# rmazzier/OpenSetGaitRecognition_PCAA

Hardware: AMD Instinct MI355X
Metric: gait sequences/sec (train step) (higher is better)
Workload: dtype bf16; 1 GPU; PCAA V4 train step (enc+dec+disc fwd/bwd, WGAN-GP, Chamfer, 2x Adam), B=64/GPU T=30 N=128 C=4 K=8, BASELINE config[1]; global_batch=64, precision=bf16, parallelism=dp1, sync_bn=False, finite_loss=True, hip_graph=False, decoder_update=fused wgrad+adam

## Files before the change

### include/pcaa_hip.h

```cpp
#ifndef PCAA_HIP_H
#define PCAA_HIP_H

#include <stddef.h>

#ifdef __cplusplus
extern "C" {
#endif

#define PCAA_ABI_VERSION 20

#define PCAA_OK 0
#define PCAA_ERR_INVALID_ARG 1
#define PCAA_ERR_LAUNCH 2

#define PCAA_F32 0
#define PCAA_BF16 1
#define PCAA_SPLIT_F16 2

#define PCAA_LAYOUT_KC 0
#define PCAA_LAYOUT_RC 1

#define PCAA_ACT_NONE 0
#define PCAA_ACT_ELU 1

const char* pcaa_last_error(void);
int pcaa_abi_version(void);

int pcaa_gemm(int math,
              const void* A, int a_dtype, int a_layout, long lda,
              const void* B, int b_dtype, int b_layout, long ldb,
              void* C, int c_dtype, long ldc,
              int M, int N, int K,
              const float* bias, double* colstats, int nrep,
              int split_k, int accumulate, void* stream);

int pcaa_gemm_num_splits(int math, int K, int split_k);
int pcaa_gemm_group_rc_f32(int n, const void* const* A, const void* const* B, void* const* C, const int* M,
                           const int* N, const int* K, const int* split_k, void* stream);
int pcaa_gemm_group_rc_f32_slabs(int n, const void* const* A, const void* const* B, void* const* slabs, const int* M,
                                 const int* N, const int* K, const int* split_k, void* stream);
int pcaa_gemm_v2_enable(int on);
int pcaa_gemm_slabs(int math,
// ... 85 lines not shown
                         float* scale, float* shift, float* mean, float* rstd, int ch, unsigned* counter);
int pcaa_bn_tail_arm_bwd(const double* stats, int nrep, long count, const float* gamma,
                         const float* mean, const float* rstd,
                         float* coef, float* dgamma, float* dbeta, int ch, unsigned* counter);
int pcaa_bn_tail_pending(void);
int pcaa_bn_tail_disarm(void);
int pcaa_bn_bwd_dy_fused(const void* da, const float* dpool, int group_rows, float pool_scale,
                         const void* y, void* dy, int dtype, const float* scale, const float* shift,
                         const float* coef, long rows, int ch, void* stream);

int pcaa_bias_act(float* y, const float* bias, int act, long rows, int cols, void* stream);
int pcaa_elu_bwd_from_out(const float* da, const float* a, float* dz, long n, void* stream);
int pcaa_colsum(const float* x, float* out, long rows, int cols, void* stream);
int pcaa_sum(const float* x, long n, float scale, float* out, void* stream);
int pcaa_rowsum(const float* x, float* out, long rows, int cols, float scale, void* stream);
int pcaa_scale_by_device_scalar(const float* x, const float* s, float* out, long n, void* stream);
int pcaa_scale_rows(const float* x, const float* s, float* out, long rows, int cols, void* stream);
int pcaa_prior_sample(const float* z0, const float* means, const long long* gt, int B, int K, int D,
                      float* z, float* onehot, void* stream);
int pcaa_pack_points(const float* src, long sb, long sc, long st, long sn,
                     float* dst, int B, int C, int T, int N, void* stream);

int pcaa_gather_rows(const void* src, long n_src_rows, long row_bytes, const long long* idx, void* dst,
                     long n_rows, int* err_flag, void* stream);

int pcaa_dtc_im2col(const float* a, float* col, int B, int T, int Cin, int dilation, void* stream);
int pcaa_dtc_col2im(const float* dcol, float* da, int B, int T, int Cin, int dilation, void* stream);

int pcaa_chamfer_fwd_bwd(const float* preds, long p_sb, long p_sc, long p_st, long p_sn,
                         const float* gts, long g_sb, long g_sc, long g_st, long g_sn,
                         int B, int T, int N, int C, float* frame_loss,
                         float* dpreds, long d_sb, long d_sc, long d_st, long d_sn,
                         float grad_scale, const float* grad_per_b, void* stream);
int pcaa_cross_entropy(const float* logits, const long long* target, int B, int K,
                       float* loss, float* dlogits, float grad_scale, long long* preds,
                       int* err_flag, void* stream);

int pcaa_disc_forward(const float* x, const float* label, int B, int K,
                      const float* W1, const float* b1, const float* W2, const float* b2,
                      const float* W3, const float* b3, float* out, void* stream);
int pcaa_disc_backward(const float* x, const float* label, int B, int K,
                       const float* W1, const float* b1, const float* W2, const float* b2,
                       const float* W3, const float* b3, const float* gout,
                       float* dx, float* dlabel,
                       float* dW1, float* db1, float* dW2, float* db2, float* dW3, float* db3,
                       float* workspace, size_t workspace_bytes, void* stream);
int pcaa_disc_backward_backward(const float* x, const float* label, int B, int K,
                                const float* W1, const float* b1, const float* W2, const float* b2,
                                const float* W3, const float* b3, const float* gout, const float* gbar,
                                float* dx2, float* dlabel2, float* dgout,
                                float* dW1, float* db1, float* dW2, float* db2, float* dW3, float* db3,
                                float* workspace, size_t workspace_bytes, void* stream);
size_t pcaa_disc_workspace_bytes(int B, int K);
int pcaa_disc_wgan_gp(const float* z, const float* fv, const float* label, const float* alphas,
                      int B, int K,
                      const float* W1, const float* b1, const float* W2, const float* b2,
                      const float* W3, const float* b3, float gp_weight, float* losses,
                      float* dW1, float* db1, float* dW2, float* db2, float* dW3, float* db3,
                      float* dz, float* workspace, size_t workspace_bytes, void* stream);

int pcaa_joint_likelihood(const float* x, const float* means, int B, int K, int D, double* lik,
                          void* stream);
int pcaa_kvote(const double* lik, const long long* preds, double threshold, int k, int n_labels,
               int n_classes, int n_windows, long long* out, void* stream);

int pcaa_skinny_supported(int M, int N, int K);
// ... 104 lines not shown
                   float* dW1, float* db1, float* dWh, float* dbh, float* dW2, float* db2, float* dWg,
                   float* dbg, float* dx4, int B, int K, void* stream);

int pcaa_gemm_split3_supported(int M, int N, int K);
int pcaa_gemm_split3(const void* A, const void* B, int layout, long lda, long ldb, float* C, long ldc, int M,
                     int N, int K, double* colstats, int nrep, float out_scale, void* stream);
int pcaa_gemm_split3_num_splits(int K, int split_k);
int pcaa_gemm_slabs_split3(const void* A, const void* B, int layout, long lda, long ldb, float* slabs,
                           long slab_stride, int M, int N, int K, int split_k, float out_scale, void* stream);
int pcaa_split_f16(const float* src, void* dst_img, long rows, int ch, int transpose, float img_scale, void* stream);
int pcaa_set_range_flag(int* dev_flag);
int pcaa_bn_act_fwd_split(const float* y, void* a_img, const float* scale, const float* shift, long rows,
                          int ch, float img_scale, void* stream);
int pcaa_bn_bwd_dy_fused_split(const float* da, const float* dpool, int group_rows, float pool_scale,
                               const float* y, void* dy_img, const float* scale, const float* shift,
                               const float* coef, long rows, int ch, float img_scale, void* stream);

int pcaa_orced_heads_supported(int B, int K, int d_in, int d_lat);
int pcaa_orced_heads_fwd(const float* x4, const float* Wmu, const float* bmu, const float* Wlv, const float* blv,
                         const float* eps, const float* Wc, const float* bc, float* mu, float* logvar, float* sup_fv,
                         float* logits, int B, int K, int d_in, int d_lat, void* stream);
int pcaa_orced_heads_bwd(const float* x4, const float* eps, const float* logvar, const float* sup_fv,
                         const float* Wmu, const float* Wlv, const float* Wc, const float* d_logits,
                         const float* d_sup, const float* d_mu, const float* d_logvar, float* ws, float* dWmu,
                         float* dbmu, float* dWlv, float* dblv, float* dWc, float* dbc, float* dx4, int B, int K,
                         int d_in, int d_lat, void* stream);
int pcaa_orced_kl(const float* mu, const float* logvar, const float* mu_k, float* loss, float* d_mu,
                  float* d_logvar, float* d_muk, float gscale, int B, int d_lat, void* stream);

int pcaa_adam_step(float* param, const float* grad, float* exp_avg, float* exp_avg_sq, long n,
                   float lr, float beta1, float beta2, float eps, int step, float grad_scale,
                   int max_blocks, void* stream);
int pcaa_adam_advance(int* step_dev, float* coef_dev, float lr, float beta1, float beta2, void* stream);
int pcaa_adam_step_dev(float* param, const float* grad, float* exp_avg, float* exp_avg_sq, long n,
                       float beta1, float beta2, float eps, const float* coef_dev, float grad_scale,
                       int max_blocks, void* stream);
int pcaa_adam_step_dev_g16(float* param, const void* grad_bf16, float* exp_avg, float* exp_avg_sq, long n,
                           float beta1, float beta2, float eps, const float* coef_dev, float grad_scale,
                           int max_blocks, void* stream);

#ifdef __cplusplus
}
#endif
#endif
```

### opensetgaitrecognition_pcaa_amd/csrc/elementwise.hip

```cpp
#include <stdarg.h>

#include "common.h"
#include "bn_tail.h"

static thread_local char g_err[512] = "";
void pcaa_set_error(const char* fmt, ...) {
  va_list ap;
  va_start(ap, fmt);
  vsnprintf(g_err, sizeof(g_err), fmt, ap);
  va_end(ap);
}
extern "C" const char* pcaa_last_error(void) { return g_err; }
static thread_local int* g_range_flag = nullptr;
int* pcaa_range_flag_ptr() { return g_range_flag; }
extern "C" int pcaa_set_range_flag(int* dev_flag) { g_range_flag = dev_flag; return PCAA_OK; }
extern "C" int pcaa_abi_version(void) { return PCAA_ABI_VERSION; }

namespace {

constexpr int ROWS_PER_BLOCK = 128;

inline bool ch_ok(int ch) {
  if (ch < 4 || ch > 1024 || (ch & 3)) return false;
  const int q = ch >> 2;
// ... 505 lines not shown
  const long stride = (long)gridDim.x * 256;
  for (long q0 = (long)blockIdx.x * 256 + threadIdx.x; q0 < nq; q0 += stride * U) {
    f32x4 pv[U], gv[U], mv[U], vv[U];
#pragma unroll
    for (int u = 0; u < U; ++u) {
      const long q = q0 + u * stride;
      if (q < nq) { pv[u] = load4(p + q * 4); gv[u] = load4(g + q * 4); mv[u] = load4(m + q * 4); vv[u] = load4(v + q * 4); }
    }
#pragma unroll
    for (int u = 0; u < U; ++u) {
      const long q = q0 + u * stride;
      if (q >= nq) break;
#pragma unroll
      for (int e = 0; e < 4; ++e) {
        float pe = pv[u][e], me = mv[u][e], ve = vv[u][e];
        adam_update(pe, me, ve, gv[u][e] * grad_scale, b1, b2, eps, step_size, inv_bc2_sqrt);
        pv[u][e] = pe; mv[u][e] = me; vv[u][e] = ve;
      }
      store4(p + q * 4, pv[u]);
      store4(m + q * 4, mv[u]);
      store4(v + q * 4, vv[u]);
    }
  }
  if (blockIdx.x == 0 && threadIdx.x < (n & 3)) {
    const long i = (nq << 2) + threadIdx.x;
    float pp = p[i], mm = m[i], vv = v[i];
    adam_update(pp, mm, vv, (float)g[i] * grad_scale, b1, b2, eps, step_size, inv_bc2_sqrt);
    m[i] = mm;
    v[i] = vv;
    p[i] = pp;
  }
}

__global__ void adam_coef_kernel(int* __restrict__ step, float* __restrict__ coef, float lr, float b1, float b2) {
  const int t = *step + 1;
  *step = t;
  const double bc1 = 1.0 - pow((double)b1, (double)t);
  const double bc2 = 1.0 - pow((double)b2, (double)t);
  coef[0] = (float)((double)lr / bc1);
  coef[1] = (float)(1.0 / sqrt(bc2));
}

inline int grid_for(long work_items, int per_block = 256, int cap = 256 * 8) {
  long g = cdiv(work_items, per_block);
  if (g < 1) g = 1;
  if (g > cap) g = cap;
  return (int)g;
}

inline int col_invariant_grid(long nquads, int qpr) {
  int a = qpr, b = 256;
  while (b) { const int t = a % b; a = b; b = t; }
  const int unit = qpr / a;
  long g = cdiv(nquads, 256);
  if (g > 2048) g = 2048;
  g = cdiv(g, unit) * unit;
  return (int)g;
}

}

extern "C" int pcaa_bn_finalize(const double* stats, int nrep, long count, const float* lin_bias,
                                const float* gamma, const float* beta, float* running_mean,
                                float* running_var, long long* num_batches_tracked, float momentum,
                                float eps, float* scale, float* shift, float* mean, float* rstd,
                                int ch, void* stream) {
  PCAA_CHECK_ARG(stats && gamma && beta && scale && shift && mean && rstd, "pcaa_bn_finalize: null pointer");
  PCAA_CHECK_ARG(nrep >= 1 && count >= 1 && ch >= 1, "pcaa_bn_finalize: bad sizes");
  PCAA_CHECK_ARG((running_mean == nullptr) == (running_var == nullptr), "pcaa_bn_finalize: running stats must come together");
  const double unbias = count > 1 ? (double)count / (double)(count - 1) : 1.0;
  hipLaunchKernelGGL(bn_finalize_kernel, dim3((unsigned)cdiv(ch, 256)), dim3(256), 0, as_stream(stream),
                     stats, nrep, 1.0 / (double)count, unbias, lin_bias, gamma, beta, running_mean,
                     running_var, num_batches_tracked, momentum, eps, scale, shift, mean, rstd, ch);
// ... 499 lines not shown
                                      int max_blocks, void* stream) {
  PCAA_CHECK_ARG(param && grad_bf16 && exp_avg && exp_avg_sq && coef_dev && n >= 1 && max_blocks >= 0,
                 "pcaa_adam_step_dev_g16: bad args");
  PCAA_CHECK_ARG(((uintptr_t)param % 16) == 0 && ((uintptr_t)grad_bf16 % 8) == 0 && ((uintptr_t)exp_avg % 16) == 0 &&
                 ((uintptr_t)exp_avg_sq % 16) == 0, "pcaa_adam_step_dev_g16: buffers must be 16-B (gradient: 8-B) aligned");
  const bf16_t* g = reinterpret_cast<const bf16_t*>(grad_bf16);
  const int cap = max_blocks > 0 ? max_blocks : 256 * 16;
  if (cap <= 1024)
    hipLaunchKernelGGL((adam_kernel<4, bf16_t>), dim3(grid_for(n >> 4, 256, cap)), dim3(256), 0, as_stream(stream), param, g,
                       exp_avg, exp_avg_sq, n, beta1, beta2, eps, 0.f, 0.f, grad_scale, coef_dev);
  else
    hipLaunchKernelGGL((adam_kernel<1, bf16_t>), dim3(grid_for(n >> 2, 256, cap)), dim3(256), 0, as_stream(stream), param, g,
                       exp_avg, exp_avg_sq, n, beta1, beta2, eps, 0.f, 0.f, grad_scale, coef_dev);
  PCAA_RETURN_LAUNCH_STATUS("pcaa_adam_step_dev_g16");
}

extern "C" int pcaa_adam_step(float* param, const float* grad, float* exp_avg, float* exp_avg_sq, long n,
                              float lr, float beta1, float beta2, float eps, int step, float grad_scale,
                              int max_blocks, void* stream) {
  PCAA_CHECK_ARG(param && grad && exp_avg && exp_avg_sq && n >= 1 && step >= 1 && max_blocks >= 0,
                 "pcaa_adam_step: bad args");
  const double bc1 = 1.0 - pow((double)beta1, (double)step);
  const double bc2 = 1.0 - pow((double)beta2, (double)step);
  return launch_adam(param, grad, exp_avg, exp_avg_sq, n, beta1, beta2, eps, (float)((double)lr / bc1),
                     (float)(1.0 / sqrt(bc2)), nullptr, grad_scale, max_blocks, stream, "pcaa_adam_step");
}

extern "C" int pcaa_adam_advance(int* step_dev, float* coef_dev, float lr, float beta1, float beta2, void* stream) {
  PCAA_CHECK_ARG(step_dev && coef_dev, "pcaa_adam_advance: bad args");
  hipLaunchKernelGGL(adam_coef_kernel, dim3(1), dim3(1), 0, as_stream(stream), step_dev, coef_dev, lr, beta1, beta2);
  PCAA_RETURN_LAUNCH_STATUS("pcaa_adam_advance");
}

extern "C" int pcaa_adam_step_dev(float* param, const float* grad, float* exp_avg, float* exp_avg_sq, long n,
                                  float beta1, float beta2, float eps, const float* coef_dev, float grad_scale,
                                  int max_blocks, void* stream) {
  PCAA_CHECK_ARG(param && grad && exp_avg && exp_avg_sq && coef_dev && n >= 1 && max_blocks >= 0,
                 "pcaa_adam_step_dev: bad args");
  return launch_adam(param, grad, exp_avg, exp_avg_sq, n, beta1, beta2, eps, 0.f, 0.f, coef_dev, grad_scale,
                     max_blocks, stream, "pcaa_adam_step_dev");
}
```

### opensetgaitrecognition_pcaa_amd/csrc/losses.hip

```cpp
#include "common.h"

namespace {

constexpr int MAXC = 8;
constexpr int CH_THREADS = 256;

__global__ __launch_bounds__(CH_THREADS) void chamfer_kernel(
    const float* __restrict__ preds, long p_sb, long p_sc, long p_st, long p_sn,
    const float* __restrict__ gts, long g_sb, long g_sc, long g_st, long g_sn,
    int T, int N, int C, float* __restrict__ frame_loss,
    float* __restrict__ dpreds, long d_sb, long d_sc, long d_st, long d_sn,
    float grad_scale, const float* __restrict__ grad_per_b) {
  extern __shared__ __attribute__((aligned(16))) float sm[];
  float* sg = sm;
  float* sp = sg + (long)N * MAXC;
  float* rg = sp + (long)N * MAXC;
  float* rp = rg + N;
  int* nn = reinterpret_cast<int*>(rp + N);
  __shared__ float red[CH_THREADS / 64];

  const int frame = blockIdx.x;
  const int b = frame / T, t = frame - b * T;
  const float* pb = preds + b * p_sb + t * p_st;
  const float* gb = gts + b * g_sb + t * g_st;
// ... 31 lines not shown
    float best = 3.4e38f;
    int bi = 0;
    for (int o = 0; o < N; ++o) {
      float dot = 0.f;
#pragma unroll
      for (int c = 0; c < MAXC; ++c) dot = fmaf(other[o * MAXC + c], v[c], dot);
      const float P = (dir1 ? (rother[o] + rme) : (rme + rother[o])) - 2.f * dot;
      if (P < best) { best = P; bi = o; }
    }
    loss += best;
    nn[item] = bi;
  }
  loss = wave_sum(loss);
  if ((threadIdx.x & 63) == 0) red[threadIdx.x >> 6] = loss;
  __syncthreads();
  if (threadIdx.x == 0) {
    float tot = 0.f;
    for (int i = 0; i < CH_THREADS / 64; ++i) tot += red[i];
    frame_loss[frame] = tot;
  }
  if (dpreds) {
    __syncthreads();
    float* db = dpreds + b * d_sb + t * d_st;
    for (int e = threadIdx.x; e < N * C; e += CH_THREADS) {
      const int c = e / N, n = e - c * N;
      const float pv = sp[n * MAXC + c];
      float g = 2.f * w * (pv - sg[nn[n] * MAXC + c]);
      for (int i = 0; i < N; ++i)
        if (nn[N + i] == n) g += 2.f * w * (pv - sg[i * MAXC + c]);
      db[c * d_sc + n * d_sn] = g;
    }
  }
}

__global__ __launch_bounds__(256) void cross_entropy_kernel(const float* __restrict__ logits,
                                                            const long long* __restrict__ target, int B,
                                                            int K, float* loss, float* dlogits,
                                                            float grad_scale, long long* preds, int* err_flag) {
  __shared__ double red[4];
  double acc = 0.0;
  for (int r = threadIdx.x; r < B; r += 256) {
    const float* x = logits + (long)r * K;
    float mx = x[0];
    for (int k = 1; k < K; ++k) mx = fmaxf(mx, x[k]);
    float se = 0.f;
    for (int k = 0; k < K; ++k) se += expf(x[k] - mx);
    const float inv = 1.f / se;
    int am = 0;
    float pbest = -1.f;
    long long tg = target ? target[r] : 0;
    if (tg < 0 || tg >= K) {
      if (err_flag) *err_flag = 1;
      tg = 0;
    }
    for (int k = 0; k < K; ++k) {
      const float pk = expf(x[k] - mx) / se;
      if (pk > pbest) { pbest = pk; am = k; }
      if (dlogits) dlogits[(long)r * K + k] = grad_scale * (expf(x[k] - mx) * inv - (k == tg ? 1.f : 0.f)) / (float)B;
    }
    if (preds) preds[r] = am;
    if (target) acc += (double)(logf(se) + mx - x[tg]);
  }
  acc = wave_sum_d(acc);
  if ((threadIdx.x & 63) == 0) red[threadIdx.x >> 6] = acc;
  __syncthreads();
  if (threadIdx.x == 0 && loss) loss[0] = (float)((red[0] + red[1] + red[2] + red[3]) / B);
}

}

extern "C" int pcaa_chamfer_fwd_bwd(const float* preds, long p_sb, long p_sc, long p_st, long p_sn,
                                    const float* gts, long g_sb, long g_sc, long g_st, long g_sn,
                                    int B, int T, int N, int C, float* frame_loss, float* dpreds,
                                    long d_sb, long d_sc, long d_st, long d_sn, float grad_scale,
                                    const float* grad_per_b, void* stream) {
  PCAA_CHECK_ARG(preds && gts && frame_loss, "pcaa_chamfer_fwd_bwd: null pointer");
  PCAA_CHECK_ARG(B >= 1 && T >= 1 && N >= 1 && C >= 1 && C <= MAXC, "pcaa_chamfer_fwd_bwd: need 1<=C<=%d (C=%d)", MAXC, C);
  const size_t lds = ((size_t)2 * N * MAXC + 4 * (size_t)N) * sizeof(float);
  PCAA_CHECK_ARG(lds <= 150 * 1024, "pcaa_chamfer_fwd_bwd: N=%d too large for one LDS tile", N);
  if (lds > 64 * 1024) {
    hipError_t e = hipFuncSetAttribute(reinterpret_cast<const void*>(chamfer_kernel),
                                       hipFuncAttributeMaxDynamicSharedMemorySize, (int)lds);
    if (e != hipSuccess) { pcaa_set_error("pcaa_chamfer_fwd_bwd: cannot raise LDS limit: %s", hipGetErrorString(e)); return PCAA_ERR_LAUNCH; }
  }
  hipLaunchKernelGGL(chamfer_kernel, dim3((unsigned)(B * T)), dim3(CH_THREADS), lds, as_stream(stream),
                     preds, p_sb, p_sc, p_st, p_sn, gts, g_sb, g_sc, g_st, g_sn, T, N, C, frame_loss,
                     dpreds, d_sb, d_sc, d_st, d_sn, grad_scale, grad_per_b);
  PCAA_RETURN_LAUNCH_STATUS("pcaa_chamfer_fwd_bwd");
}

extern "C" int pcaa_cross_entropy(const float* logits, const long long* target, int B, int K, float* loss,
                                  float* dlogits, float grad_scale, long long* preds, int* err_flag,
                                  void* stream) {
  PCAA_CHECK_ARG(logits && B >= 1 && K >= 1, "pcaa_cross_entropy: bad args");
  PCAA_CHECK_ARG(target || (!loss && !dlogits), "pcaa_cross_entropy: loss/grad need targets");
  hipLaunchKernelGGL(cross_entropy_kernel, dim3(1), dim3(256), 0, as_stream(stream), logits, target, B, K,
                     loss, dlogits, grad_scale, preds, err_flag);
  PCAA_RETURN_LAUNCH_STATUS("pcaa_cross_entropy");
}
```

### opensetgaitrecognition_pcaa_amd/ops.py

```python
import ctypes
import os

import torch

from . import _lib
from ._lib import ACT_ELU, ACT_NONE, KC, PCAA_BF16, PCAA_F32, RC, check

PCAA_SPLIT_F16 = 2

NREP = 16
BN_EPS = 1e-5
BN_MOMENTUM = 0.1


def _p(t):
    return None if t is None else t.data_ptr()


_raw_stream = getattr(torch._C, "_cuda_getCurrentRawStream", None)
_raw_device = getattr(torch._C, "_cuda_getDevice", None)


def _s():
    if _raw_stream is not None and _raw_device is not None:
# ... 1428 lines not shown
    D = sup_fv.shape[1]
    k, n_votes, n_runs = int(k), int(n_votes), run_start.numel() - 1
    if (sup_fv.shape[0] != nw or means.shape[1] != D or win_stream.numel() != nw or win_j.numel() != nw
            or vote_pos.numel() != nw or k < 1 or tuple(hist_lik.shape) != tuple(hist_pred.shape)
            or hist_lik.shape[1] != k or not 0 <= n_votes <= nw or not (1 <= n_runs <= nw or nw == 0)):
        raise ValueError("stream_score: shapes do not describe one tick")
    dev = logits.device
    preds = torch.empty(nw, dtype=torch.int64, device=dev)
    lik = torch.empty(nw, dtype=torch.float64, device=dev)
    votes = torch.empty(n_votes, dtype=torch.int64, device=dev)
    if nw:
        check(_lib.load().pcaa_stream_score(
            _p(logits), _p(sup_fv), _p(means), _p(run_start), n_runs, _p(win_stream), _p(win_j), _p(vote_pos), nw, K, D,
            means.shape[0], ctypes.c_double(float(threshold)), k, int(n_labels), int(n_classes), _p(hist_lik),
            _p(hist_pred), hist_lik.shape[0], _p(preds), _p(lik), _p(votes) if n_votes else None, n_votes, _s()),
            "pcaa_stream_score")
    return preds, lik, votes


def dtc_im2col(a, B, T, Cin, d):
    _chk(a, "im2col.a", torch.float32, 2)
    col = torch.empty((B * T, 3 * Cin), dtype=torch.float32, device=a.device)
    check(_lib.load().pcaa_dtc_im2col(_p(a), _p(col), B, T, Cin, d, _s()), "pcaa_dtc_im2col")
    return col


def dtc_col2im(dcol, B, T, Cin, d):
    _chk(dcol, "col2im.dcol", torch.float32, 2)
    da = torch.empty((B * T, Cin), dtype=torch.float32, device=dcol.device)
    check(_lib.load().pcaa_dtc_col2im(_p(dcol), _p(da), B, T, Cin, d, _s()), "pcaa_dtc_col2im")
    return da


def chamfer(preds, gts, want_grad, grad_scale=1.0, grad_per_b=None):
    for t, nm in ((preds, "preds"), (gts, "gts")):
        if not t.is_cuda or t.dtype != torch.float32 or t.dim() != 4:
            raise RuntimeError(f"chamfer: {nm} must be a 4-D float32 tensor on the HIP device")
    if preds.shape != gts.shape:
        raise ValueError("chamfer: shape mismatch")
    B, C, T, N = preds.shape
    fl = torch.empty((B, T), dtype=torch.float32, device=preds.device)
    dp = torch.empty((B, C, T, N), dtype=torch.float32, device=preds.device) if want_grad else None
    ds = dp.stride() if want_grad else (0, 0, 0, 0)
    ps, gs = preds.stride(), gts.stride()
    check(_lib.load().pcaa_chamfer_fwd_bwd(_p(preds), ps[0], ps[1], ps[2], ps[3], _p(gts), gs[0], gs[1], gs[2], gs[3],
                                           B, T, N, C, _p(fl), _p(dp), ds[0], ds[1], ds[2], ds[3],
                                           float(grad_scale), _p(grad_per_b), _s()), "pcaa_chamfer_fwd_bwd")
    return fl, dp


def cross_entropy(logits, target=None, want_loss=True, want_grad=False, grad_scale=1.0, want_preds=False,
                  err_flag=None):
    _chk(logits, "ce.logits", torch.float32, 2)
    B, K = logits.shape
    if target is not None:
        _chk(target, "ce.target", torch.int64, 1)
        if target.shape[0] != B:
            raise ValueError(f"cross_entropy: {target.shape[0]} targets for {B} rows of logits")
        if err_flag is None:
            lo, hi = int(target.min().item()), int(target.max().item())
            if lo < 0 or hi >= K:
                raise IndexError(f"cross_entropy: target {lo if lo < 0 else hi} is out of bounds for {K} classes")
        else:
            _chk(err_flag, "ce.err_flag", torch.int32)
    dev = logits.device
    loss = torch.empty((), dtype=torch.float32, device=dev) if (want_loss and target is not None) else None
    dl = torch.empty_like(logits) if want_grad else None
    pr = torch.empty(B, dtype=torch.int64, device=dev) if want_preds else None
    check(_lib.load().pcaa_cross_entropy(_p(logits), _p(target), B, K, _p(loss), _p(dl), float(grad_scale), _p(pr),
                                         _p(err_flag) if target is not None else None, _s()),
          "pcaa_cross_entropy")
    return loss, dl, pr


def orced_heads_fwd(x4, Wmu, bmu, Wlv, blv, eps, Wc, bc):
    for t, nm in ((x4, "x4"), (Wmu, "Wmu"), (Wlv, "Wlv"), (eps, "eps"), (Wc, "Wc")):
        _chk(t, f"orced_heads_fwd.{nm}", torch.float32, 2)
    B, d_in = x4.shape
    L, K = Wmu.shape[0], Wc.shape[0]
    lib = _lib.load()
# ... 114 lines not shown
        raise ValueError("disc_wgan_gp: shapes")
    dev = z.device
    losses = torch.empty(2, dtype=torch.float32, device=dev) if losses_out is None else _chk(losses_out, "wgan.losses_out", torch.float32)
    if losses.numel() != 2:
        raise ValueError("disc_wgan_gp: losses_out must hold 2 floats")
    grads = grads_out if grads_out is not None else [torch.empty_like(p) for p in params]
    ws = disc_workspace(B, K, dev)
    dz = torch.empty_like(z) if want_dz else None
    check(_lib.load().pcaa_disc_wgan_gp(_p(z), _p(fv), _p(label), _p(alphas), B, K, *[_p(p) for p in params],
                                        float(gp_weight), _p(losses), *[_p(g) for g in grads], _p(dz), _p(ws),
                                        ws.numel() * 4, _s()), "pcaa_disc_wgan_gp")
    if want_dz:
        return losses, grads, dz
    return losses, grads


def adam_step_(p, g, m, v, lr, b1, b2, eps, step, grad_scale=1.0, max_blocks=0):
    for t, nm in ((p, "p"), (g, "g"), (m, "m"), (v, "v")):
        _chk(t, f"adam.{nm}", torch.float32)
    n = p.numel()
    if not (g.numel() == n and m.numel() == n and v.numel() == n):
        raise ValueError("adam_step_: size mismatch")
    check(_lib.load().pcaa_adam_step(_p(p), _p(g), _p(m), _p(v), n, float(lr), float(b1), float(b2), float(eps),
                                     int(step), float(grad_scale), int(max_blocks), _s()), "pcaa_adam_step")


def adam_advance_(step_dev, coef_dev, lr, b1, b2):
    _chk(step_dev, "adam.step_dev", torch.int32)
    _chk(coef_dev, "adam.coef_dev", torch.float32)
    if step_dev.numel() != 1 or coef_dev.numel() != 2:
        raise ValueError("adam_advance_: step_dev is int32[1], coef_dev float32[2]")
    check(_lib.load().pcaa_adam_advance(_p(step_dev), _p(coef_dev), float(lr), float(b1), float(b2), _s()),
          "pcaa_adam_advance")


def adam_step_dev_(p, g, m, v, b1, b2, eps, coef_dev, grad_scale=1.0, max_blocks=0):
    for nm, t in (("p", p), ("g", g), ("m", m), ("v", v)):
        _chk(t, f"adam.{nm}", torch.float32)
    _chk(coef_dev, "adam.coef_dev", torch.float32)
    n = p.numel()
    if not (g.numel() == m.numel() == v.numel() == n) or coef_dev.numel() != 2:
        raise ValueError("adam_step_dev_: size mismatch")
    check(_lib.load().pcaa_adam_step_dev(_p(p), _p(g), _p(m), _p(v), n, float(b1), float(b2), float(eps),
                                         _p(coef_dev), float(grad_scale), int(max_blocks), _s()),
          "pcaa_adam_step_dev")


def adam_step_dev_g16_(p, g16, m, v, b1, b2, eps, coef_dev, grad_scale=1.0, max_blocks=0):
    for nm, t in (("p", p), ("m", m), ("v", v)):
        _chk(t, f"adam_g16.{nm}", torch.float32)
    _chk(g16, "adam_g16.g", torch.bfloat16)
    _chk(coef_dev, "adam_g16.coef_dev", torch.float32)
    n = p.numel()
    if not (g16.numel() == m.numel() == v.numel() == n) or coef_dev.numel() != 2:
        raise ValueError("adam_step_dev_g16_: size mismatch")
    check(_lib.load().pcaa_adam_step_dev_g16(_p(p), _p(g16), _p(m), _p(v), n, float(b1), float(b2), float(eps),
                                             _p(coef_dev), float(grad_scale), int(max_blocks), _s()),
          "pcaa_adam_step_dev_g16")


def heads_supported(B, K, d_in, d_sup, d_head, d_proj, backward):
    return bool(_lib.load().pcaa_heads_supported(int(B), int(K), int(d_in), int(d_sup), int(d_head), int(d_proj),
                                                 1 if backward else 0))


def heads_fwd(x4, W1, b1, Wh, bh, W2, b2, Wg=None, bg=None):
# ... 160 lines not shown
```

### opensetgaitrecognition_pcaa_amd/train.py

```python
import itertools
import math
import os
import pickle

import numpy as np
import torch

from . import constants
from . import dist as pdist
from . import functional as F_hip
from . import ops
from ._lib import ACT_ELU
from .models import CGDecoder, CGDiscriminator, CGEncoder, GaussianMeanLearner
from .utils import sample_distant_points, save_model

_ALIGN = 64


_SIDE_STREAMS = {}


_SIDE_ADAM_AT = os.environ.get("PCAA_SIDE_ADAM_AT", "dec_bwd")


# ... 159 lines not shown
        self.fused_exact = bool(fused_decoder_update)
        if grad_compress not in (None, "bf16"):
            raise ValueError("grad_compress must be None or 'bf16'")
        self.grad_compress = grad_compress
        self.comm = {"collectives": 0, "payload_bytes": 0}
        self.time_comm = False
        self.comm_events = []
        self._step_events = None
        if variant not in ("v4", "base", "v1", "v3"):
            raise ValueError(f"PCAATrainer: unknown variant {variant!r}")
        head = variant in ("v4", "v1")
        self.learn_centroids = bool(learn_centroids) and variant == "v1"
        self.encoder = CGEncoder(n_out_labels=self.K, use_projection_head=head, nmax_points=self.N).to(self.device).float()
        self.decoder = None if variant == "v3" else \
            CGDecoder(input_dim=self.L * 2 if head else self.L, nmax_points=self.N).to(self.device).float()
        if variant != "v1":
            self.discriminator = CGDiscriminator(self.K).to(self.device).float()
        self.decoder_projection_head = self.discriminator_projection_head = self.mean_learner = None
        if variant == "v1":
            self.decoder_projection_head = torch.nn.Sequential(
                torch.nn.Linear(self.L, self.L * 2), torch.nn.ELU()).to(self.device).float()
            self.discriminator = CGDiscriminator(self.K).to(self.device).float()
            self.mean_learner = GaussianMeanLearner(self.K).to(self.device).float()
        elif head:
            self.decoder_projection_head = torch.nn.Sequential(
                torch.nn.Linear(self.L, self.L * 2), torch.nn.ELU()).to(self.device).float()
            self.discriminator_projection_head = torch.nn.Sequential(
                torch.nn.Linear(self.L * 2, self.L), torch.nn.ELU()).to(self.device).float()
        self.discriminator_means = None
        self._flat_ready = False
        self.gradless_ranges = []
        self._graphs = {}
        self._err = torch.zeros(1, dtype=torch.int32, device=self.device)
        self._sup_split = False

    def set_prior_means(self, means):
        self.discriminator_means = means.float().to(self.device).contiguous()

    def sample_prior_means(self):
        self.set_prior_means(sample_distant_points(dimension=self.L, n=self.K, min_dist=10, sphere_radius=10))
        return self.discriminator_means

    def _sync_bn(self):
        return F_hip.sync_bn_group(self._sync_bn_group)

    def betas_g(self):
        c = self.cfg
        return (c["B1"], c["B1"]) if self.variant == "v3" else (c["B1"], c["B2"])

    def modules(self):
        d = {"E": self.encoder, "D": self.discriminator}
        if self.decoder is not None:
            d = {"E": self.encoder, "G": self.decoder, "D": self.discriminator}
        if self.decoder_projection_head is not None:
            d["GPH"] = self.decoder_projection_head
        if self.discriminator_projection_head is not None:
            d["DPH"] = self.discriminator_projection_head
        if self.mean_learner is not None:
            d["ML"] = self.mean_learner
        return d

    def finalize(self):
        g_named = [("E." + n, p) for n, p in self.encoder.named_parameters()]
        if self.decoder_projection_head is not None:
            g_named += [("GPH." + n, p) for n, p in self.decoder_projection_head.named_parameters()]
        if self.decoder is not None:
# ... 124 lines not shown
        for m in self.modules().values():
            m.eval()

    def _count(self, nbytes, kind="allreduce"):
        self.comm["collectives"] += 1
        self.comm["payload_bytes"] += int(nbytes)
        self.comm[kind + "_bytes"] = self.comm.get(kind + "_bytes", 0) + int(nbytes)

    def _allreduce(self, t, async_op=False):
        if self._collective() and t.numel():
            in_dec = (t.data_ptr() >= self.flat_g.g.data_ptr() + 4 * self._dec_start
                      and t.data_ptr() < self.flat_g.g.data_ptr() + 4 * self.flat_g.total)
            off = (t.data_ptr() - self.flat_g.g.data_ptr()) // 4 if in_dec else -1
            if self.grad_compress == "bf16" and in_dec and (t.numel() >= self._COMPRESS_MIN or off in self._g16_direct):
                g16 = self._g16[off:off + t.numel()]
                if off not in self._g16_direct:
                    g16.copy_(t)
                self._count(2 * t.numel())
                work = self._xchg.all_reduce(g16, async_op=async_op)
                if not async_op:
                    t.copy_(g16)
                    return None
                return _CompressedWork(work, t, g16)
            assert off not in self._g16_direct, "a bf16-direct gradient bucket reached the fp32 all-reduce"
            self._count(t.numel() * t.element_size())
            return self._xchg.all_reduce(t, async_op=async_op)
        return None

    def _collective(self):
        return self._xchg is not None and (self.world > 1 or self._force_collectives)

    def _advance_g(self, supervise):
        b1, b2 = self.betas_g()
        self.flat_g.advance(self.cfg["LR"], b1, b2)
        if supervise:
            self.flat_g.sup_count.advance(self.cfg["LR"], b1, b2)
        else:
            self._sup_split = True

    def _adam_g(self, lo, hi, supervise, gs, max_blocks=0):
        b1, b2 = self.betas_g()
        lr, fg = self.cfg["LR"], self.flat_g
        a, b = max(lo, self._sup_range[0]), min(hi, self._sup_range[1])
        if a >= b or (supervise and not self._sup_split):
            fg.adam(lr, b1, b2, grad_scale=gs, lo=lo, hi=hi, advance=False, max_blocks=max_blocks)
            return
        fg.adam(lr, b1, b2, grad_scale=gs, lo=lo, hi=a, advance=False, max_blocks=max_blocks)
        if supervise:
            fg.adam(lr, b1, b2, grad_scale=gs, lo=a, hi=b, advance=False, count=fg.sup_count)
        fg.adam(lr, b1, b2, grad_scale=gs, lo=b, hi=hi, advance=False, max_blocks=max_blocks)

    def _w16_active(self, mode, B, collective):
        if (self.decoder is None or not self.fused_decoder_update or collective or self._side is None or mode != "bf16"
                or os.environ.get("PCAA_DEC_W16", "0") != "1"):
            return {}
        return {i: t for i, t in self._dec_fused.items() if F_hip._skinny(mode, B, t[2].shape[0], t[2].shape[1])}

    def _refresh_w16(self, mode, B, collective):
        images = {}
        if self.decoder is None:
            return images
        params = self.decoder.dense_layers()
        active = self._w16_active(mode, B, collective)
        for i, t in self._dec_fused.items():
            if i not in active:
                if i in self._dec_w16:
                    self._dec_w16[i][1] = None
                continue
            Wv = t[2]
            ent = self._dec_w16.get(i)
# ... 80 lines not shown
            for t in outs:
                t.record_stream(self._aux)
            with ops.on_stream(self._aux):
                self._aux.wait_event(fork)
                d_losses, loss_g, dsup = critic_branch(outs)
                joined = torch.cuda.Event()
                joined.record(self._aux)
        else:
            d_losses, loss_g, dsup = critic_branch()

        if self.variant == "v3":
            if joined is not None:
                ops.current_stream().wait_event(joined)
            F_hip.set_wgrad_stream(self._wg)
            try:
                F_hip.encoder_backward(enc, st, dlogits if supervise else None, dsup, gout=self._enc_grads)
            finally:
                F_hip.set_wgrad_stream(None)
            if self._wg is not None:
                ops.current_stream().wait_stream(self._wg)
            self._allreduce(self.flat_g.g)
            self._advance_g(supervise)
            self._adam_g(0, self.flat_g.total, supervise, gs)
            tot = loss_g + (sup_loss if supervise else 0.0)
            return {"d_loss": d_losses[0], "gp": d_losses[1], "rec_loss": None, "loss_g": loss_g,
                    "sup_loss": sup_loss, "tot_loss": tot, "preds": preds, "out_labels": logits, "sup_fvs": sup_fv}

        hproj = st.hproj if self.decoder_projection_head is not None else sup_fv
        w16 = self._refresh_w16(mode, B, self._collective())
        rec, acts = F_hip.decoder_forward(dec, hproj, mode, images=w16)
        F_hip.mark("dec_fwd")
        rec4 = rec.view(B, self.C, self.T, self.N)
        inv_bt = 1.0 / (B * self.T)
        frame_loss, drec = ops.chamfer(rec4, pcs, want_grad=True, grad_scale=inv_bt)
        rec_loss = ops.total(frame_loss, inv_bt)

        F_hip.mark("chamfer")
        F_hip.set_wgrad_stream(self._wg)
        if joined is not None and self.decoder_projection_head is None:
            ops.current_stream().wait_event(joined)
            joined = None
        dh = None
        collective = self._collective()
        early_buckets = []
        layer_hook = None
        zero = self._zero and collective and self._side is not None
        if zero:
            pass
        elif collective and self._wg is not None:
            fg = self.flat_g

            def layer_hook(layer):
                if layer < 2:
                    return
                lo = fg.offsets[fg.names.index(f"G.dense{layer}.weight")]
                nxt = f"G.dense{layer + 1}.weight"
                hi = fg.offsets[fg.names.index(nxt)] if nxt in fg.names else fg.total
                self._wg.wait_stream(ops.current_stream())
                with ops.on_stream(self._wg):
                    early_buckets.append((lo, hi, self._allreduce(fg.g[lo:hi], async_op=True)))

        updates, fused_ranges, deferred = None, [], []
        exact_dec = mode in ("fp32", "fp16x3")
        if (self.fused_decoder_update and not collective and self._side is not None
                and (mode == "bf16" or (self.fused_exact and exact_dec))):
            for layer, (lo, hi, Wv, mv, vv) in self._dec_fused.items():
                if F_hip._skinny(mode, B, Wv.shape[0], Wv.shape[1]) or F_hip._skinny_exact(mode, B, Wv.shape[0], Wv.shape[1]):
                    updates = updates or {}
# ... 569 lines not shown
```

Measured before the change: 12050 sequences/s.

## Add specialized Chamfer kernel with fused total reduction and paired Adam advance

Adds a Chamfer forward/backward kernel specialized for C=4/5 and N<=256. It holds points and squared norms in LDS, uses a norm-expansion distance in the nearest-neighbour search, and has the last block reduce all frame losses into the scalar total through an atomic ticket, which removes the separate total kernel. It also merges the two Adam coefficient-advance launches into one kernel when supervised. The risks are the expanded-distance formula changing numerics slightly and the ticket/last-block pattern relying on correct memory ordering.

Result: no change. 12050 sequences/s (-0.0%).

```diff
diff --git a/include/pcaa_hip.h b/include/pcaa_hip.h
--- a/include/pcaa_hip.h
+++ b/include/pcaa_hip.h
@@ -7,7 +7,7 @@
 extern "C" {
 #endif
 
-#define PCAA_ABI_VERSION 20
+#define PCAA_ABI_VERSION 21
 
 #define PCAA_OK 0
 #define PCAA_ERR_INVALID_ARG 1
@@ -159,6 +159,17 @@
                          int B, int T, int N, int C, float* frame_loss,
                          float* dpreds, long d_sb, long d_sc, long d_st, long d_sn,
                          float grad_scale, const float* grad_per_b, void* stream);
+int pcaa_chamfer_fwd_bwd_generic(const float* preds, long p_sb, long p_sc, long p_st, long p_sn,
+                                 const float* gts, long g_sb, long g_sc, long g_st, long g_sn,
+                                 int B, int T, int N, int C, float* frame_loss,
+                                 float* dpreds, long d_sb, long d_sc, long d_st, long d_sn,
+                                 float grad_scale, const float* grad_per_b, void* stream);
+int pcaa_chamfer_fwd_bwd_total(const float* preds, long p_sb, long p_sc, long p_st, long p_sn,
+                               const float* gts, long g_sb, long g_sc, long g_st, long g_sn,
+                               int B, int T, int N, int C, float* frame_loss,
+                               float* dpreds, long d_sb, long d_sc, long d_st, long d_sn,
+                               float grad_scale, const float* grad_per_b,
+                               float total_scale, float* total, int* ticket, void* stream);
 int pcaa_cross_entropy(const float* logits, const long long* target, int B, int K,
                        float* loss, float* dlogits, float grad_scale, long long* preds,
                        int* err_flag, void* stream);
@@ -329,6 +340,8 @@
                    float lr, float beta1, float beta2, float eps, int step, float grad_scale,
                    int max_blocks, void* stream);
 int pcaa_adam_advance(int* step_dev, float* coef_dev, float lr, float beta1, float beta2, void* stream);
+int pcaa_adam_advance_pair(int* step_dev_a, float* coef_dev_a, int* step_dev_b, float* coef_dev_b,
+                           float lr, float beta1, float beta2, void* stream);
 int pcaa_adam_step_dev(float* param, const float* grad, float* exp_avg, float* exp_avg_sq, long n,
                        float beta1, float beta2, float eps, const float* coef_dev, float grad_scale,
                        int max_blocks, void* stream);
diff --git a/opensetgaitrecognition_pcaa_amd/csrc/elementwise.hip b/opensetgaitrecognition_pcaa_amd/csrc/elementwise.hip
--- a/opensetgaitrecognition_pcaa_amd/csrc/elementwise.hip
+++ b/opensetgaitrecognition_pcaa_amd/csrc/elementwise.hip
@@ -561,13 +561,23 @@
   }
 }
 
-__global__ void adam_coef_kernel(int* __restrict__ step, float* __restrict__ coef, float lr, float b1, float b2) {
+__device__ __forceinline__ void adam_coef_advance(int* step, float* coef, float lr, float b1, float b2) {
   const int t = *step + 1;
   *step = t;
   const double bc1 = 1.0 - pow((double)b1, (double)t);
   const double bc2 = 1.0 - pow((double)b2, (double)t);
   coef[0] = (float)((double)lr / bc1);
   coef[1] = (float)(1.0 / sqrt(bc2));
+}
+
+__global__ void adam_coef_kernel(int* __restrict__ step, float* __restrict__ coef, float lr, float b1, float b2) {
+  adam_coef_advance(step, coef, lr, b1, b2);
+}
+
+__global__ void adam_coef_pair_kernel(int* step_a, float* coef_a, int* step_b, float* coef_b, float lr, float b1,
+                                      float b2) {
+  if (threadIdx.x == 0) adam_coef_advance(step_a, coef_a, lr, b1, b2);
+  else adam_coef_advance(step_b, coef_b, lr, b1, b2);
 }
 
 inline int grid_for(long work_items, int per_block = 256, int cap = 256 * 8) {
@@ -1133,6 +1143,15 @@
   PCAA_RETURN_LAUNCH_STATUS("pcaa_adam_advance");
 }
 
+extern "C" int pcaa_adam_advance_pair(int* step_dev_a, float* coef_dev_a, int* step_dev_b, float* coef_dev_b, float lr,
+                                      float beta1, float beta2, void* stream) {
+  PCAA_CHECK_ARG(step_dev_a && coef_dev_a && step_dev_b && coef_dev_b, "pcaa_adam_advance_pair: bad args");
+  PCAA_CHECK_ARG(step_dev_a != step_dev_b && coef_dev_a != coef_dev_b, "pcaa_adam_advance_pair: the two counts must differ");
+  hipLaunchKernelGGL(adam_coef_pair_kernel, dim3(1), dim3(2), 0, as_stream(stream), step_dev_a, coef_dev_a, step_dev_b,
+                     coef_dev_b, lr, beta1, beta2);
+  PCAA_RETURN_LAUNCH_STATUS("pcaa_adam_advance_pair");
+}
+
 extern "C" int pcaa_adam_step_dev(float* param, const float* grad, float* exp_avg, float* exp_avg_sq, long n,
                                   float beta1, float beta2, float eps, const float* coef_dev, float grad_scale,
                                   int max_blocks, void* stream) {
diff --git a/opensetgaitrecognition_pcaa_amd/csrc/losses.hip b/opensetgaitrecognition_pcaa_amd/csrc/losses.hip
--- a/opensetgaitrecognition_pcaa_amd/csrc/losses.hip
+++ b/opensetgaitrecognition_pcaa_amd/csrc/losses.hip
@@ -87,6 +87,175 @@
     }
   }
 }
+
+constexpr int CF_MAXN = 256;
+constexpr int CF_TILE = 128;
+
+template <int C>
+__global__ __launch_bounds__(256) void chamfer_fast_kernel(
+    const float* __restrict__ preds, long p_sb, long p_sc, long p_st, long p_sn,
+    const float* __restrict__ gts, long g_sb, long g_sc, long g_st, long g_sn,
+    int T, int N, float* frame_loss,
+    float* __restrict__ dpreds, long d_sb, long d_sc, long d_st, long d_sn,
+    float grad_scale, const float* __restrict__ grad_per_b,
+    float total_scale, float* __restrict__ total, unsigned* __restrict__ ticket) {
+  constexpr int RS = C == 4 ? 4 : 8;
+  extern __shared__ __attribute__((aligned(16))) float sm[];
+  const int NP = (N + 3) & ~3;
+  float* sg = sm;
+  float* sp = sg + NP * RS;
+  float* rg = sp + NP * RS;
+  float* rp = rg + NP;
+  int* nn = reinterpret_cast<int*>(rp + NP);
+  float* bestv = reinterpret_cast<float*>(nn + 2 * NP);
+  double* red = reinterpret_cast<double*>(bestv + 2 * NP);
+  int* flag = reinterpret_cast<int*>(red + 16);
+
+  const int tid = threadIdx.x, nthreads = blockDim.x;
+  const int frame = blockIdx.x;
+  const int b = frame / T, t = frame - b * T;
+  const float* pb = preds + b * p_sb + t * p_st;
+  const float* gb = gts + b * g_sb + t * g_st;
+
+  for (int n = tid; n < NP; n += nthreads) {
+    if (n < N) {
+      float a = 0.f, q = 0.f;
+#pragma unroll
+      for (int c = 0; c < C; ++c) {
+        const float gv = gb[c * g_sc + n * g_sn], pv = pb[c * p_sc + n * p_sn];
+        sg[n * RS + c] = gv;
+        sp[n * RS + c] = pv;
+        a = fmaf(gv, gv, a);
+        q = fmaf(pv, pv, q);
+      }
+      rg[n] = a;
+      rp[n] = q;
+    } else {
+      nn[NP + n] = -1;
+    }
+  }
+  __syncthreads();
+
+  {
+    const int wave = __builtin_amdgcn_readfirstlane(tid >> 6), lane = tid & 63;
+    const int nwd = nthreads >> 7;
+    const bool dir1 = wave < nwd;
+    const int base = (dir1 ? wave : wave - nwd) * CF_TILE;
+    const float* mine = dir1 ? sp : sg;
+    const float* rmine = dir1 ? rp : rg;
+    const float* other = dir1 ? sg : sp;
+    const float* rother = dir1 ? rg : rp;
+    const int i0 = base + lane, i1 = i0 + 64;
+    const int m0 = min(i0, N - 1), m1 = min(i1, N - 1);
+    float v0[C], v1[C];
+#pragma unroll
+    for (int c = 0; c < C; ++c) { v0[c] = mine[m0 * RS + c]; v1[c] = mine[m1 * RS + c]; }
+    const float r0 = rmine[m0], r1 = rmine[m1];
+    float best0 = 3.4e38f, best1 = 3.4e38f;
+    int bi0 = 0, bi1 = 0;
+#pragma unroll 4
+    for (int o = 0; o < N; ++o) {
+      float row[C];
+      if constexpr (C == 4) {
+        const f32x4 r = *reinterpret_cast<const f32x4*>(other + o * RS);
+        row[0] = r.x; row[1] = r.y; row[2] = r.z; row[3] = r.w;
+      } else {
+#pragma unroll
+        for (int c = 0; c < C; ++c) row[c] = other[o * RS + c];
+      }
+      const float ro = rother[o];
+      float d0 = 0.f, d1 = 0.f;
+#pragma unroll
+      for (int c = 0; c < C; ++c) { d0 = fmaf(row[c], v0[c], d0); d1 = fmaf(row[c], v1[c], d1); }
+      const float P0 = (ro + r0) - 2.f * d0;
+      const float P1 = (ro + r1) - 2.f * d1;
+      if (P0 < best0) { best0 = P0; bi0 = o; }
+      if (P1 < best1) { best1 = P1; bi1 = o; }
+    }
+    const int off = dir1 ? 0 : NP, ioff = dir1 ? 0 : N;
+    if (i0 < N) { nn[off + i0] = bi0; bestv[ioff + i0] = best0; }
+    if (i1 < N) { nn[off + i1] = bi1; bestv[ioff + i1] = best1; }
+  }
+  __syncthreads();
+
+  if (tid < 64) {
+    float tot = 0.f;
+#pragma unroll
+    for (int k = 0; k < 4; ++k) {
+      const int v = k * 64 + tid;
+      float loss = 0.f;
+      if (v < 2 * N) loss += bestv[v];
+      if (v + 256 < 2 * N) loss += bestv[v + 256];
+      loss = wave_sum(loss);
+      tot += loss;
+    }
+    if (tid == 0) {
+      if (ticket != nullptr) {
+        __hip_atomic_store(frame_loss + frame, tot, __ATOMIC_RELAXED, __HIP_MEMORY_SCOPE_AGENT);
+        asm volatile("s_waitcnt vmcnt(0)" ::: "memory");
+        const unsigned prev = __hip_atomic_fetch_add(ticket, 1u, __ATOMIC_RELAXED, __HIP_MEMORY_SCOPE_AGENT);
+        *flag = prev == gridDim.x - 1 ? 1 : 0;
+      } else {
+        frame_loss[frame] = tot;
+      }
+    }
+  }
+
+  if (dpreds) {
+    const float tw = 2.f * (grad_scale * (grad_per_b ? grad_per_b[b] : 1.f));
+    float* db = dpreds + b * d_sb + t * d_st;
+    for (int n = tid; n < N; n += nthreads) {
+      float pv[C], g[C];
+      const int j = nn[n];
+#pragma unroll
+      for (int c = 0; c < C; ++c) {
+        pv[c] = sp[n * RS + c];
+        g[c] = tw * (pv[c] - sg[j * RS + c]);
+      }
+      for (int i = 0; i < NP; i += 4) {
+        const int4 q = *reinterpret_cast<const int4*>(nn + NP + i);
+        const int qq[4] = {q.x, q.y, q.z, q.w};
+#pragma unroll
+        for (int u = 0; u < 4; ++u) {
+          if (qq[u] == n) {
+#pragma unroll
+            for (int c = 0; c < C; ++c) g[c] = __builtin_fmaf(tw, pv[c] - sg[(i + u) * RS + c], g[c]);
+          }
+        }
+      }
+#pragma unroll
+      for (int c = 0; c < C; ++c) db[c * d_sc + n * d_sn] = g[c];
+    }
+  }
+
+  if (ticket == nullptr) return;
+  __syncthreads();
+  if (*flag == 0) return;
+  __builtin_amdgcn_fence(__ATOMIC_ACQUIRE, "wavefront");
+  const long nframes = gridDim.x;
+  for (int k = 0; k * nthreads < 1024; ++k) {
+    const int v = tid + k * nthreads;
+    double acc = 0.0;
+    for (long i = v; i < nframes; i += 1024)
+      acc += (double)__hip_atomic_load(frame_loss + i, __ATOMIC_RELAXED, __HIP_MEMORY_SCOPE_AGENT);
+    acc = wave_sum_d(acc);
+    if ((tid & 63) == 0) red[v >> 6] = acc;
+  }
+  __syncthreads();
+  if (tid == 0) {
+    __hip_atomic_store(ticket, 0u, __ATOMIC_RELAXED, __HIP_MEMORY_SCOPE_AGENT);
+    double s = 0.0;
+    for (int i = 0; i < 16; ++i) s += red[i];
+    total[0] = (float)(s * (double)total_scale);
+  }
+}
+
+size_t chamfer_fast_lds(int N, int C) {
+  const size_t NP = ((size_t)N + 3) & ~(size_t)3, RS = C == 4 ? 4 : 8;
+  return (2 * NP * RS + 2 * NP + 4 * NP) * sizeof(float) + 16 * sizeof(double) + 16;
+}
+
+bool chamfer_fast_ok(int N, int C) { return (C == 4 || C == 5) && N <= CF_MAXN; }
 
 __global__ __launch_bounds__(256) void cross_entropy_kernel(const float* __restrict__ logits,
                                                             const long long* __restrict__ target, int B,
@@ -124,24 +293,85 @@
 
 }
 
+static int chamfer_generic(const float* preds, long p_sb, long p_sc, long p_st, long p_sn,
+                           const float* gts, long g_sb, long g_sc, long g_st, long g_sn,
+                           int B, int T, int N, int C, float* frame_loss, float* dpreds,
+                           long d_sb, long d_sc, long d_st, long d_sn, float grad_scale,
+                           const float* grad_per_b, void* stream, const char* who) {
+  PCAA_CHECK_ARG(preds && gts && frame_loss, "%s: null pointer", who);
+  PCAA_CHECK_ARG(B >= 1 && T >= 1 && N >= 1 && C >= 1 && C <= MAXC, "%s: need 1<=C<=%d (C=%d)", who, MAXC, C);
+  const size_t lds = ((size_t)2 * N * MAXC + 4 * (size_t)N) * sizeof(float);
+  PCAA_CHECK_ARG(lds <= 150 * 1024, "%s: N=%d too large for one LDS tile", who, N);
+  if (lds > 64 * 1024) {
+    hipError_t e = hipFuncSetAttribute(reinterpret_cast<const void*>(chamfer_kernel),
+                                       hipFuncAttributeMaxDynamicSharedMemorySize, (int)lds);
+    if (e != hipSuccess) { pcaa_set_error("%s: cannot raise LDS limit: %s", who, hipGetErrorString(e)); return PCAA_ERR_LAUNCH; }
+  }
+  hipLaunchKernelGGL(chamfer_kernel, dim3((unsigned)(B * T)), dim3(CH_THREADS), lds, as_stream(stream),
+                     preds, p_sb, p_sc, p_st, p_sn, gts, g_sb, g_sc, g_st, g_sn, T, N, C, frame_loss,
+                     dpreds, d_sb, d_sc, d_st, d_sn, grad_scale, grad_per_b);
+  PCAA_RETURN_LAUNCH_STATUS(who);
+}
+
+static int chamfer_fast(const float* preds, long p_sb, long p_sc, long p_st, long p_sn,
+                        const float* gts, long g_sb, long g_sc, long g_st, long g_sn,
+                        int B, int T, int N, int C, float* frame_loss, float* dpreds,
+                        long d_sb, long d_sc, long d_st, long d_sn, float grad_scale,
+                        const float* grad_per_b, float total_scale, float* total, int* ticket, void* stream,
+                        const char* who) {
+  PCAA_CHECK_ARG(preds && gts && frame_loss, "%s: null pointer", who);
+  PCAA_CHECK_ARG(B >= 1 && T >= 1 && N >= 1 && chamfer_fast_ok(N, C), "%s: bad shape", who);
+  const dim3 grid((unsigned)(B * T)), block(N <= CF_TILE ? 128 : 256);
+  const size_t lds = chamfer_fast_lds(N, C);
+  unsigned* tk = total ? reinterpret_cast<unsigned*>(ticket) : nullptr;
+  if (C == 4)
+    hipLaunchKernelGGL(chamfer_fast_kernel<4>, grid, block, lds, as_stream(stream), preds, p_sb, p_sc, p_st, p_sn, gts,
+                       g_sb, g_sc, g_st, g_sn, T, N, frame_loss, dpreds, d_sb, d_sc, d_st, d_sn, grad_scale, grad_per_b,
+                       total_scale, total, tk);
+  else
+    hipLaunchKernelGGL(chamfer_fast_kernel<5>, grid, block, lds, as_stream(stream), preds, p_sb, p_sc, p_st, p_sn, gts,
+                       g_sb, g_sc, g_st, g_sn, T, N, frame_loss, dpreds, d_sb, d_sc, d_st, d_sn, grad_scale, grad_per_b,
+                       total_scale, total, tk);
+  PCAA_RETURN_LAUNCH_STATUS(who);
+}
+
 extern "C" int pcaa_chamfer_fwd_bwd(const float* preds, long p_sb, long p_sc, long p_st, long p_sn,
                                     const float* gts, long g_sb, long g_sc, long g_st, long g_sn,
                                     int B, int T, int N, int C, float* frame_loss, float* dpreds,
                                     long d_sb, long d_sc, long d_st, long d_sn, float grad_scale,
                                     const float* grad_per_b, void* stream) {
-  PCAA_CHECK_ARG(preds && gts && frame_loss, "pcaa_chamfer_fwd_bwd: null pointer");
-  PCAA_CHECK_ARG(B >= 1 && T >= 1 && N >= 1 && C >= 1 && C <= MAXC, "pcaa_chamfer_fwd_bwd: need 1<=C<=%d (C=%d)", MAXC, C);
-  const size_t lds = ((size_t)2 * N * MAXC + 4 * (size_t)N) * sizeof(float);
-  PCAA_CHECK_ARG(lds <= 150 * 1024, "pcaa_chamfer_fwd_bwd: N=%d too large for one LDS tile", N);
-  if (lds > 64 * 1024) {
-    hipError_t e = hipFuncSetAttribute(reinterpret_cast<const void*>(chamfer_kernel),
-                                       hipFuncAttributeMaxDynamicSharedMemorySize, (int)lds);
-    if (e != hipSuccess) { pcaa_set_error("pcaa_chamfer_fwd_bwd: cannot raise LDS limit: %s", hipGetErrorString(e)); return PCAA_ERR_LAUNCH; }
-  }
-  hipLaunchKernelGGL(chamfer_kernel, dim3((unsigned)(B * T)), dim3(CH_THREADS), lds, as_stream(stream),
-                     preds, p_sb, p_sc, p_st, p_sn, gts, g_sb, g_sc, g_st, g_sn, T, N, C, frame_loss,
-                     dpreds, d_sb, d_sc, d_st, d_sn, grad_scale, grad_per_b);
-  PCAA_RETURN_LAUNCH_STATUS("pcaa_chamfer_fwd_bwd");
+  if (chamfer_fast_ok(N, C))
+    return chamfer_fast(preds, p_sb, p_sc, p_st, p_sn, gts, g_sb, g_sc, g_st, g_sn, B, T, N, C, frame_loss, dpreds,
+                        d_sb, d_sc, d_st, d_sn, grad_scale, grad_per_b, 0.f, nullptr, nullptr, stream,
+                        "pcaa_chamfer_fwd_bwd");
+  return chamfer_generic(preds, p_sb, p_sc, p_st, p_sn, gts, g_sb, g_sc, g_st, g_sn, B, T, N, C, frame_loss, dpreds,
+                         d_sb, d_sc, d_st, d_sn, grad_scale, grad_per_b, stream, "pcaa_chamfer_fwd_bwd");
+}
+
+extern "C" int pcaa_chamfer_fwd_bwd_generic(const float* preds, long p_sb, long p_sc, long p_st, long p_sn,
+                                            const float* gts, long g_sb, long g_sc, long g_st, long g_sn,
+                                            int B, int T, int N, int C, float* frame_loss, float* dpreds,
+                                            long d_sb, long d_sc, long d_st, long d_sn, float grad_scale,
+                                            const float* grad_per_b, void* stream) {
+  return chamfer_generic(preds, p_sb, p_sc, p_st, p_sn, gts, g_sb, g_sc, g_st, g_sn, B, T, N, C, frame_loss, dpreds,
+                         d_sb, d_sc, d_st, d_sn, grad_scale, grad_per_b, stream, "pcaa_chamfer_fwd_bwd_generic");
+}
+
+extern "C" int pcaa_chamfer_fwd_bwd_total(const float* preds, long p_sb, long p_sc, long p_st, long p_sn,
+                                          const float* gts, long g_sb, long g_sc, long g_st, long g_sn,
+                                          int B, int T, int N, int C, float* frame_loss, float* dpreds,
+                                          long d_sb, long d_sc, long d_st, long d_sn, float grad_scale,
+                                          const float* grad_per_b, float total_scale, float* total, int* ticket,
+                                          void* stream) {
+  PCAA_CHECK_ARG(total && ticket, "pcaa_chamfer_fwd_bwd_total: null pointer");
+  if (chamfer_fast_ok(N, C))
+    return chamfer_fast(preds, p_sb, p_sc, p_st, p_sn, gts, g_sb, g_sc, g_st, g_sn, B, T, N, C, frame_loss, dpreds,
+                        d_sb, d_sc, d_st, d_sn, grad_scale, grad_per_b, total_scale, total, ticket, stream,
+                        "pcaa_chamfer_fwd_bwd_total");
+  const int rc = chamfer_generic(preds, p_sb, p_sc, p_st, p_sn, gts, g_sb, g_sc, g_st, g_sn, B, T, N, C, frame_loss,
+                                 dpreds, d_sb, d_sc, d_st, d_sn, grad_scale, grad_per_b, stream,
+                                 "pcaa_chamfer_fwd_bwd_total");
+  return rc != PCAA_OK ? rc : pcaa_sum(frame_loss, (long)B * T, total_scale, total, stream);
 }
 
 extern "C" int pcaa_cross_entropy(const float* logits, const long long* target, int B, int K, float* loss,
diff --git a/opensetgaitrecognition_pcaa_amd/ops.py b/opensetgaitrecognition_pcaa_amd/ops.py
--- a/opensetgaitrecognition_pcaa_amd/ops.py
+++ b/opensetgaitrecognition_pcaa_amd/ops.py
@@ -1484,7 +1484,7 @@
     return da
 
 
-def chamfer(preds, gts, want_grad, grad_scale=1.0, grad_per_b=None):
+def chamfer(preds, gts, want_grad, grad_scale=1.0, grad_per_b=None, total_scale=None, ticket=None, generic=False):
     for t, nm in ((preds, "preds"), (gts, "gts")):
         if not t.is_cuda or t.dtype != torch.float32 or t.dim() != 4:
             raise RuntimeError(f"chamfer: {nm} must be a 4-D float32 tensor on the HIP device")
@@ -1495,9 +1495,18 @@
     dp = torch.empty((B, C, T, N), dtype=torch.float32, device=preds.device) if want_grad else None
     ds = dp.stride() if want_grad else (0, 0, 0, 0)
     ps, gs = preds.stride(), gts.stride()
-    check(_lib.load().pcaa_chamfer_fwd_bwd(_p(preds), ps[0], ps[1], ps[2], ps[3], _p(gts), gs[0], gs[1], gs[2], gs[3],
-                                           B, T, N, C, _p(fl), _p(dp), ds[0], ds[1], ds[2], ds[3],
-                                           float(grad_scale), _p(grad_per_b), _s()), "pcaa_chamfer_fwd_bwd")
+    args = (_p(preds), ps[0], ps[1], ps[2], ps[3], _p(gts), gs[0], gs[1], gs[2], gs[3],
+            B, T, N, C, _p(fl), _p(dp), ds[0], ds[1], ds[2], ds[3], float(grad_scale), _p(grad_per_b))
+    if total_scale is not None:
+        if generic:
+            raise ValueError("chamfer: the generic entry has no fused total")
+        _chk(ticket, "chamfer.ticket", torch.int32)
+        tot = torch.empty((), dtype=torch.float32, device=preds.device)
+        check(_lib.load().pcaa_chamfer_fwd_bwd_total(*args, float(total_scale), _p(tot), _p(ticket), _s()),
+              "pcaa_chamfer_fwd_bwd_total")
+        return fl, dp, tot
+    name = "pcaa_chamfer_fwd_bwd_generic" if generic else "pcaa_chamfer_fwd_bwd"
+    check(getattr(_lib.load(), name)(*args, _s()), name)
     return fl, dp
 
 
@@ -1678,6 +1687,16 @@
         raise ValueError("adam_advance_: step_dev is int32[1], coef_dev float32[2]")
     check(_lib.load().pcaa_adam_advance(_p(step_dev), _p(coef_dev), float(lr), float(b1), float(b2), _s()),
           "pcaa_adam_advance")
+
+
+def adam_advance_pair_(step_a, coef_a, step_b, coef_b, lr, b1, b2):
+    for st, cf in ((step_a, coef_a), (step_b, coef_b)):
+        _chk(st, "adam.step_dev", torch.int32)
+        _chk(cf, "adam.coef_dev", torch.float32)
+        if st.numel() != 1 or cf.numel() != 2:
+            raise ValueError("adam_advance_pair_: step_dev is int32[1], coef_dev float32[2]")
+    check(_lib.load().pcaa_adam_advance_pair(_p(step_a), _p(coef_a), _p(step_b), _p(coef_b), float(lr), float(b1),
+                                             float(b2), _s()), "pcaa_adam_advance_pair")
 
 
 def adam_step_dev_(p, g, m, v, b1, b2, eps, coef_dev, grad_scale=1.0, max_blocks=0):
diff --git a/opensetgaitrecognition_pcaa_amd/train.py b/opensetgaitrecognition_pcaa_amd/train.py
--- a/opensetgaitrecognition_pcaa_amd/train.py
+++ b/opensetgaitrecognition_pcaa_amd/train.py
@@ -215,6 +215,7 @@
         self.gradless_ranges = []
         self._graphs = {}
         self._err = torch.zeros(1, dtype=torch.int32, device=self.device)
+        self._chamfer_ticket = torch.zeros(1, dtype=torch.int32, device=self.device)
         self._sup_split = False
 
     def set_prior_means(self, means):
@@ -405,10 +406,13 @@
 
     def _advance_g(self, supervise):
         b1, b2 = self.betas_g()
-        self.flat_g.advance(self.cfg["LR"], b1, b2)
         if supervise:
-            self.flat_g.sup_count.advance(self.cfg["LR"], b1, b2)
+            main, sup = self.flat_g.count, self.flat_g.sup_count
+            main.step += 1
+            sup.step += 1
+            ops.adam_advance_pair_(main.step_dev, main.coef_dev, sup.step_dev, sup.coef_dev, self.cfg["LR"], b1, b2)
         else:
+            self.flat_g.advance(self.cfg["LR"], b1, b2)
             self._sup_split = True
 
     def _adam_g(self, lo, hi, supervise, gs, max_blocks=0):
@@ -555,8 +559,8 @@
         F_hip.mark("dec_fwd")
         rec4 = rec.view(B, self.C, self.T, self.N)
         inv_bt = 1.0 / (B * self.T)
-        frame_loss, drec = ops.chamfer(rec4, pcs, want_grad=True, grad_scale=inv_bt)
-        rec_loss = ops.total(frame_loss, inv_bt)
+        frame_loss, drec, rec_loss = ops.chamfer(rec4, pcs, want_grad=True, grad_scale=inv_bt, total_scale=inv_bt,
+                                                 ticket=self._chamfer_ticket)
 
         F_hip.mark("chamfer")
         F_hip.set_wgrad_stream(self._wg)
```
